# JacksonCampolattaro/spectrogram-rs

Hardware: AMD Instinct MI355X
Metric: STFT frames/sec (4096-pt, hop 256) (higher is better)
Workload: dtype f32

## Files before the change

### bindings/rust/sgx_sys.rs

```rust
use std::os::raw::{c_char, c_int, c_void};

#[repr(C)]
pub struct SgxConfig {
    pub struct_size: u32,
    pub sample_rate: f32, pub period: f32, pub stride: f32,
    pub window_samples: u32, pub hop_samples: u32, pub channels: u32, pub rows: u32,
    pub f_min: f64, pub f_max: f64,
    pub min_db: f32, pub max_db: f32,
    pub interp: u32, pub lut_index_mode: u32,
    pub device: i32, pub flags: u32,
}
#[repr(C)] pub struct SgxCtx { _private: [u8; 0] }
#[repr(C)] pub struct SgxFbank { _private: [u8; 0] }

extern "C" {
    pub fn sgx_config_init(cfg: *mut SgxConfig) -> c_int;
    pub fn sgx_create(cfg: *const SgxConfig, out: *mut *mut SgxCtx) -> c_int;
    pub fn sgx_destroy(ctx: *mut SgxCtx);
    pub fn sgx_last_error(ctx: *const SgxCtx) -> *const c_char;
    pub fn sgx_num_frames(ctx: *const SgxCtx, n_samples: usize) -> usize;
    pub fn sgx_process_one(ctx: *mut SgxCtx, h_lr: *const f32, n_avail: usize, h_out: *mut f32) -> c_int;
    pub fn sgx_stft_batch(ctx: *mut SgxCtx, d_pcm: *const f32, n_samples: usize, first_frame: usize,
                          max_frames: usize, d_mags: *mut f32, n_out: *mut usize) -> c_int;
    pub fn sgx_stft_batch_f16(ctx: *mut SgxCtx, d_pcm: *const f32, n_samples: usize, first_frame: usize,
// ... 28 lines not shown
                            power: u32, out_fbank: *mut *mut SgxFbank) -> c_int;
    pub fn sgx_fbank_destroy(fbank: *mut SgxFbank);
    pub fn sgx_fbank_filters(fbank: *const SgxFbank) -> u32;
    pub fn sgx_fbank_batch(fbank: *mut SgxFbank, d_pcm: *const f32, n_samples: usize, first_frame: usize, max_frames: usize,
                           d_out: *mut f32, n_out: *mut usize) -> c_int;
    pub fn sgx_fbank_mags(fbank: *mut SgxFbank, d_mags: *const f32, n_columns: usize, d_out: *mut f32) -> c_int;
    pub fn sgx_fbank_fused(fbank: *const SgxFbank) -> c_int;
    pub fn sgx_fbank_cross_batch(fbank: *mut SgxFbank, d_pcm: *const f32, n_samples: usize, first_frame: usize, max_frames: usize,
                                 d_out: *mut f32, n_out: *mut usize) -> c_int;
    pub fn sgx_fbank_cross_spec(fbank: *mut SgxFbank, d_spec: *const f32, n_columns: usize, d_out: *mut f32) -> c_int;
    pub fn sgx_fbank_cross_fused(fbank: *const SgxFbank) -> c_int;
    pub fn sgx_mel_weights(sample_rate: f64, window_samples: u32, n_mels: u32, f_min: f64, f_max: f64, scale: u32, norm: u32,
                           h_first: *mut u32, h_count: *mut u32, h_weights: *mut f32, n_weights: *mut usize) -> c_int;
    pub fn sgx_set_gradient(ctx: *mut SgxCtx, h_rgb: *const u8, n: u32, stereo: c_int) -> c_int;
    pub fn sgx_set_gradient_fn(ctx: *mut SgxCtx, eval: extern "C" fn(f64, *mut u8, *mut c_void), user: *mut c_void,
                               stereo: c_int) -> c_int;
    pub fn sgx_set_builtin_scheme(ctx: *mut SgxCtx, name: *const c_char, stereo: c_int) -> c_int;
    pub fn sgx_lookup_table(ctx: *mut SgxCtx, resolution: u32, h_out: *mut f32) -> c_int;
    pub fn sgx_sync(ctx: *mut SgxCtx) -> c_int;
    pub fn sgx_set_cu_limit(ctx: *mut SgxCtx, n: u32) -> c_int;
    pub fn sgx_cu_limit(ctx: *const SgxCtx) -> u32;
    pub fn sgx_set_run_claim(ctx: *mut SgxCtx, static_sixteenths: u32, chunk_jobs: u32) -> c_int;
    pub fn sgx_run_claim(ctx: *const SgxCtx, n_frames: usize, static_sixteenths: *mut u32, chunk_jobs: *mut u32) -> c_int;
}
extern "C" {
    pub fn hipMalloc(p: *mut *mut c_void, bytes: usize) -> c_int;
    pub fn hipFree(p: *mut c_void) -> c_int;
    pub fn hipMemcpy(dst: *mut c_void, src: *const c_void, bytes: usize, kind: c_int) -> c_int;
}
pub const HIP_MEMCPY_HOST_TO_DEVICE: c_int = 1;
pub const HIP_MEMCPY_DEVICE_TO_HOST: c_int = 2;
pub const SGX_FLAG_PAIRED_FRAMES: u32 = 1024;
pub const SGX_FLAG_COMPLEX_MONO: u32 = 512;
pub const SGX_FLAG_LARGE_TRANSFORM: u32 = 4096;
pub const SGX_MEL_HTK: u32 = 0;
pub const SGX_MEL_SLANEY: u32 = 1;
pub const SGX_MEL_NORM_NONE: u32 = 0;
pub const SGX_MEL_NORM_SLANEY: u32 = 1;
pub const SGX_LIVE_BANDS: c_int = 3;
```

### include/sgx.h

```cpp
#ifndef SGX_H
#define SGX_H

#include <stddef.h>
#include <stdint.h>

#ifdef __cplusplus
extern "C" {
#endif

#if defined(__GNUC__)
#define SGX_API __attribute__((visibility("default")))
#else
#define SGX_API
#endif

typedef enum sgx_status {
    SGX_OK = 0,
    SGX_ERR_INVALID_ARG = -1,
    SGX_ERR_UNSUPPORTED = -2,
    SGX_ERR_HIP = -3,
    SGX_ERR_NOMEM = -4,
    SGX_ERR_NO_DEVICE = -5
} sgx_status;

// ... 49 lines not shown


SGX_API const char *sgx_version(void);

SGX_API int sgx_config_init(sgx_config *cfg);

SGX_API int sgx_create(const sgx_config *cfg, sgx_ctx **out_ctx);
SGX_API void sgx_destroy(sgx_ctx *ctx);

SGX_API const char *sgx_last_error(const sgx_ctx *ctx);

SGX_API int sgx_query(const sgx_ctx *ctx, sgx_info *out);

SGX_API size_t sgx_num_frames(const sgx_ctx *ctx, size_t n_samples);

SGX_API int sgx_set_stream(sgx_ctx *ctx, void *stream);
SGX_API int sgx_sync(sgx_ctx *ctx);

SGX_API int sgx_set_cu_limit(sgx_ctx *ctx, uint32_t n);
SGX_API uint32_t sgx_cu_limit(const sgx_ctx *ctx);

SGX_API int sgx_set_run_claim(sgx_ctx *ctx, uint32_t static_sixteenths, uint32_t chunk_jobs);
SGX_API int sgx_run_claim(const sgx_ctx *ctx, size_t n_frames, uint32_t *static_sixteenths, uint32_t *chunk_jobs);


SGX_API int sgx_stft_batch(sgx_ctx *ctx, const float *d_pcm, size_t n_samples, size_t first_frame,
                           size_t max_frames, float *d_mags, size_t *n_out);

SGX_API int sgx_stft_batch_complex(sgx_ctx *ctx, const float *d_pcm, size_t n_samples, size_t first_frame,
                                   size_t max_frames, float *d_spec, size_t *n_out);

SGX_API int sgx_istft_batch(sgx_ctx *ctx, const float *d_spec, size_t n_frames, size_t first_sample,
                            size_t max_samples, float *d_pcm, size_t *n_out);
SGX_API int sgx_istft_supported(const sgx_ctx *ctx);

SGX_API int sgx_stft_batch_f16(sgx_ctx *ctx, const float *d_pcm, size_t n_samples, size_t first_frame,
                               size_t max_frames, void *d_mags_f16, size_t *n_out);

SGX_API int sgx_process_one(sgx_ctx *ctx, const float *h_lr, size_t n_avail, float *h_out);


SGX_API int sgx_render_batch(sgx_ctx *ctx, const float *d_pcm, size_t n_samples, size_t first_frame,
                             size_t max_frames, uint8_t *d_rgba, size_t *n_out);

SGX_API int sgx_render_mags(sgx_ctx *ctx, const float *d_mags, size_t n_columns, uint8_t *d_rgba);

// ... 108 lines not shown
```

### spectrogram_rs_amd/_lib.py

```python
from __future__ import annotations

import ctypes as C
import os

_HERE = os.path.dirname(os.path.abspath(__file__))
LIB_PATH = os.environ.get("SGX_LIB", os.path.join(_HERE, "libsgx.so"))

SGX_OK = 0
SGX_ERR_INVALID_ARG = -1
SGX_ERR_UNSUPPORTED = -2
SGX_ERR_HIP = -3
SGX_ERR_NOMEM = -4
SGX_ERR_NO_DEVICE = -5

INTERP_CUBIC, INTERP_COSINE = 0, 1
LUT_FLOOR_N, LUT_ROUND_NM1 = 0, 1
FLAG_FORCE_GENERIC = 1
FLAG_NO_FUSED_RENDER = 4
FLAG_LUT_WALK = 64
FLAG_MIXED_GENERIC = 256
FLAG_COMPLEX_MONO = 512
FLAG_PAIRED_FRAMES = 1024
FLAG_LARGE_TRANSFORM = 4096
LIVE_MAGS, LIVE_MAGS_F16, LIVE_RGBA, LIVE_BANDS = 0, 1, 2, 3
# ... 44 lines not shown
        ("stft_kernel", C.c_uint32),
        ("render_path", C.c_uint32),
        ("mags_bytes_per_frame", C.c_uint64),
        ("rgba_bytes_per_frame", C.c_uint64),
    ]


_vp, _sz = C.c_void_p, C.c_size_t
_ctx = C.c_void_p
SIGNATURES = [
    ("sgx_version", C.c_char_p, []),
    ("sgx_config_init", C.c_int, [C.POINTER(sgx_config)]),
    ("sgx_create", C.c_int, [C.POINTER(sgx_config), C.POINTER(_ctx)]),
    ("sgx_destroy", None, [_ctx]),
    ("sgx_last_error", C.c_char_p, [_ctx]),
    ("sgx_query", C.c_int, [_ctx, C.POINTER(sgx_info)]),
    ("sgx_num_frames", _sz, [_ctx, _sz]),
    ("sgx_set_stream", C.c_int, [_ctx, _vp]),
    ("sgx_sync", C.c_int, [_ctx]),
    ("sgx_set_cu_limit", C.c_int, [_ctx, C.c_uint32]),
    ("sgx_cu_limit", C.c_uint32, [_ctx]),
    ("sgx_set_run_claim", C.c_int, [_ctx, C.c_uint32, C.c_uint32]),
    ("sgx_run_claim", C.c_int, [_ctx, _sz, C.POINTER(C.c_uint32), C.POINTER(C.c_uint32)]),
    ("sgx_stft_batch", C.c_int, [_ctx, _vp, _sz, _sz, _sz, _vp, C.POINTER(_sz)]),
    ("sgx_stft_batch_f16", C.c_int, [_ctx, _vp, _sz, _sz, _sz, _vp, C.POINTER(_sz)]),
    ("sgx_stft_batch_complex", C.c_int, [_ctx, _vp, _sz, _sz, _sz, _vp, C.POINTER(_sz)]),
    ("sgx_istft_batch", C.c_int, [_ctx, _vp, _sz, _sz, _sz, _vp, C.POINTER(_sz)]),
    ("sgx_istft_supported", C.c_int, [_ctx]),
    ("sgx_process_one", C.c_int, [_ctx, _vp, _sz, _vp]),
    ("sgx_render_batch", C.c_int, [_ctx, _vp, _sz, _sz, _sz, _vp, C.POINTER(_sz)]),
    ("sgx_render_mags", C.c_int, [_ctx, _vp, _sz, _vp]),
    ("sgx_magnitude_in", C.c_int, [_ctx, _vp, _sz, _vp, C.c_uint32, _vp]),
    ("sgx_bands_batch", C.c_int, [_ctx, _vp, _sz, _sz, _sz, _vp, C.POINTER(_sz)]),
    ("sgx_bands_fused", C.c_int, [_ctx]),
    ("sgx_bands_peak_batch", C.c_int, [_ctx, _vp, _sz, _sz, _sz, _sz, _vp, C.POINTER(_sz)]),
    ("sgx_bands_peak_fused", C.c_int, [_ctx]),
    ("sgx_psd_batch", C.c_int, [_ctx, _vp, _sz, _sz, _sz, _sz, _vp, C.POINTER(_sz)]),
    ("sgx_csd_batch", C.c_int, [_ctx, _vp, _sz, _sz, _sz, _sz, _vp, C.POINTER(_sz)]),
    ("sgx_psd_mags", C.c_int, [_ctx, _vp, _sz, _sz, _vp, C.POINTER(_sz)]),
    ("sgx_csd_spec", C.c_int, [_ctx, _vp, _sz, _sz, _vp, C.POINTER(_sz)]),
    ("sgx_psd_fused", C.c_int, [_ctx]),
    ("sgx_csd_fused", C.c_int, [_ctx]),
    ("sgx_render_bands", C.c_int, [_ctx, _vp, _sz, _vp]),
    ("sgx_fbank_create", C.c_int, [_ctx, C.c_uint32, _vp, _vp, _vp, C.c_uint32, C.POINTER(_vp)]),
    ("sgx_fbank_destroy", None, [_vp]),
    ("sgx_fbank_filters", C.c_uint32, [_vp]),
# ... 69 lines not shown
```

### spectrogram_rs_amd/csrc/run_claim.hpp

```cpp
#pragma once

namespace sgx {

struct RunClaim {
    unsigned long long per;
    unsigned long long pool_begin;
    unsigned long long n_chunks;
    unsigned long long chunk;
};
struct JobRun { unsigned long long begin, end; };

inline RunClaim run_claim(unsigned long long n_jobs, unsigned long long blocks, unsigned static_sixteenths, unsigned long long chunk_jobs)
{
    RunClaim r;
    r.per = (n_jobs / 16 * static_sixteenths + n_jobs % 16 * static_sixteenths / 16) / blocks;
    r.pool_begin = blocks * r.per;
    r.chunk = chunk_jobs < 1 ? 1 : chunk_jobs;
    r.n_chunks = (n_jobs - r.pool_begin + r.chunk - 1) / r.chunk;
    return r;
}
inline JobRun static_run(const RunClaim &r, unsigned long long block) { return {block * r.per, (block + 1) * r.per}; }
inline JobRun claimed_run(const RunClaim &r, unsigned long long n_jobs, unsigned long long i)
{
    if (i >= r.n_chunks) return {n_jobs, n_jobs};
    const unsigned long long b = r.pool_begin + i * r.chunk, left = n_jobs - b;
    return {b, b + (left < r.chunk ? left : r.chunk)};
}

constexpr unsigned kClaimAutoSixteenths = 12, kClaimAutoChunk = 8;
constexpr unsigned long long kClaimMinStatic = 64;
inline bool run_claim_engages(unsigned long long n_jobs, unsigned long long blocks)
{
    return run_claim(n_jobs, blocks, kClaimAutoSixteenths, kClaimAutoChunk).per >= kClaimMinStatic;
}
inline bool run_claim_valid(unsigned static_sixteenths, unsigned chunk_jobs)
{
    if (chunk_jobs == 0) return static_sixteenths == 0 || static_sixteenths == 16;
    return static_sixteenths <= 16 && chunk_jobs <= (1u << 20);
}

}
```

### spectrogram_rs_amd/csrc/sgx_internal.hpp

```cpp
#pragma once

#include <hip/hip_runtime.h>

#include <cstdint>
#include <array>
#include <memory>
#include <string>
#include <vector>

#include "../../include/sgx.h"
#include "device_buffer.hpp"
#include "unit_root.hpp"

namespace sgx {

#ifdef __HIPCC__
typedef float sgx_f2v __attribute__((ext_vector_type(2)));
__device__ __forceinline__ float2 cubic_pair(float2 y0, float2 y1, float2 y2, float2 y3, float mu, float mu2, float mu3)
{
    const sgx_f2v Y0 = {y0.x, y0.y}, Y1 = {y1.x, y1.y}, Y2 = {y2.x, y2.y}, Y3 = {y3.x, y3.y};
    const sgx_f2v a0 = ((Y3 - Y2) - Y0) + Y1;
    const sgx_f2v a1 = (Y0 - Y1) - a0;
    const sgx_f2v a2 = Y2 - Y0;
    const sgx_f2v r = ((a0 * mu3) + (a1 * mu2)) + ((a2 * mu) + Y1);
// ... 107 lines not shown
    sgx::TablesPtr<sgx::blu::BluTables> blu;
    sgx::TablesPtr<sgx::mix::MixTables> mix;
    sgx::TablesPtr<sgx::w48::W48Tables> w4800;
    sgx::TablesPtr<sgx::wgr::RealTables> real;
    sgx::TablesPtr<sgx::mix::ChirpTables> chz;
    sgx::TablesPtr<sgx::w16k::TablesW> w16k;
    sgx::TablesPtr<sgx::large::LargeTables> large;
    sgx::TablesPtr<sgx::istft::ITables> istft;

    sgx::DeviceBuffer<float> d_ws_mags;
    sgx::DeviceBuffer<float> d_one_in, d_one_out;
    sgx::DeviceBuffer<unsigned long long> d_cksum;
    std::vector<float> bands_key;
    sgx::DeviceBuffer<sgx::RowEntry> d_band_rows;
    sgx::DeviceBuffer<sgx::SampleEntry> d_band_samples;
    sgx::DeviceBuffer<float> d_levels;
    sgx::DeviceBuffer<double> d_psd_carry;

    unsigned long long palette_gen = 0;

    int n_cu = 256;
    int n_cu_device = 256;
    uint32_t claim_sixteenths = 0, claim_chunk = 0;
    size_t lds_optin = 64 * 1024;
    mutable std::vector<std::pair<std::array<size_t, 3>, int>> occupancy_cache;
    std::vector<struct sgx_view *> views;
    std::vector<struct sgx_image *> images;
    std::vector<struct sgx_fbank *> fbanks;

    std::string err;

    ~sgx_ctx();
};

namespace sgx {

enum class Out { kMags, kMagsF16, kComplex, kRgba, kBands, kPeak, kFbank, kFbankCross, kPsd, kCsd };
struct StftCall {
    const float *pcm;
    uint32_t channels, pairs;
    size_t first, n, total;
    void *out;
    Out kind;
    size_t peak_group;
    const struct sgx_fbank *bank = nullptr;
};
// ... 88 lines not shown
```

### spectrogram_rs_amd/csrc/stft4096_real.hip

```cpp
#include <cmath>
#include <type_traits>

#include "run_claim.hpp"
#include "stft4096_wg.hpp"

namespace sgx {

namespace wgr {

using wg::kBufComplex;
using wg::kLdsBytes;
using wg::kLdsBytesRender;
using wg::kM;
using wg::kS1;
using wg::kS2;
using wg::kW;
using wg::lds_barrier;
using wg::lds_read_alone;
using wg::lds_cfloat2;
using wg::lds_ptr;
using wg::pcm_rsrc;
using wg::u32x2;
using wg::u32x4;

// ... 117 lines not shown
        win[2 * a] = p.window[2 * t_p1 + 512 * a] * (1.0f / 2048.0f);
        win[2 * a + 1] = p.window[2 * t_p1 + 512 * a + 1] * (1.0f / 2048.0f);
    }
    float2 tw1[8];
#pragma unroll
    for (int q = 1; q < 8; ++q) tw1[q] = p.tw1[q * 256 + t_p1];
    const int F = tid >> 7, u = tid & 127;
    float2 twu[8];
#pragma unroll
    for (int q = 0; q < 8; ++q) twu[q] = p.twu[q * 128 + u];
    const int g2 = tid >> 4, t0_2 = tid & 15;
    const int cbase2 = (g2 >> 3) * 128 + (g2 & 7);
    __syncthreads();

#ifdef SGX_VARIANT_SKIP_LAST_JOB
    constexpr bool CLAIM = false;
#else
    constexpr bool CLAIM = !FUSED;
#endif
    const bool claiming = CLAIM && p.claim_counter != nullptr;
    unsigned long long *claim_word = reinterpret_cast<unsigned long long *>(tw2 + 256);
    unsigned long long job_begin = (unsigned long long)blockIdx.x * p.jobs_per_block;
    unsigned long long job_end = job_begin + p.jobs_per_block;
    if (job_end > p.n_jobs) job_end = p.n_jobs;
#ifdef SGX_VARIANT_SKIP_LAST_JOB
    if (job_end > job_begin + 1) --job_end;
#endif
    if (job_begin >= job_end && !claiming) return;

    auto samples_from = [&](unsigned long long first) {
        const unsigned long long left = first < p.stream_samples ? (p.stream_samples - first) * 4 : 0;
        const unsigned long long addr = (unsigned long long)(p.pcm + (first < p.stream_samples ? first : 0));
        const uint32_t lo = __builtin_amdgcn_readfirstlane((uint32_t)addr), hi = __builtin_amdgcn_readfirstlane((uint32_t)(addr >> 32));
        const int records = __builtin_amdgcn_readfirstlane((int)(left < 0x7fffffffull ? left : 0x7fffffffull));
        return __builtin_amdgcn_make_buffer_rsrc(reinterpret_cast<void *>(((unsigned long long)hi << 32) | lo), 0, records, 0x00020000);
    };
    auto columns_from = [&](unsigned long long col0) { return samples_from(2 * col0); };
    auto column = [&](__amdgpu_buffer_rsrc_t r, int byte_offset) {
        const u32x2 v = __builtin_amdgcn_raw_buffer_load_b64(r, t_p1 * 8, byte_offset, 0);
        return make_float2(__uint_as_float(v.x), __uint_as_float(v.y));
    };
    float2 R[8];
    float2 L;
    auto load_pair = [&](unsigned long long fa_) {
        const __amdgpu_buffer_rsrc_t r0 = samples_from(fa_ * p.H), r1 = samples_from((fa_ + 1) * p.H);
#pragma unroll
// ... 339 lines not shown
    for (int q = 0; q < 8; ++q)
        for (int tt = 0; tt < 256; ++tt) tw1[q * 256 + tt] = unit_root2((unsigned long long)tt * q, 2048);
    for (int q = 0; q < 16; ++q)
        for (int t0 = 0; t0 < 16; ++t0) tw2[q * 16 + t0] = unit_root2((unsigned long long)t0 * q, 256);
    for (int q3 = 0; q3 < 8; ++q3)
        for (int uu = 0; uu < 128; ++uu) twu[q3 * 128 + uu] = unit_root2((unsigned long long)(uu + 128 * q3), 4096);
    twu[0] = unit_root2(1024, 4096);
    hipError_t e = t->d_tw1.upload(tw1);
    if (e == hipSuccess) e = t->d_tw2.upload(tw2);
    if (e == hipSuccess) e = t->d_twu.upload(twu);
    if (e == hipSuccess) e = t->d_claim.alloc(1);
    if (e == hipSuccess) c->real = std::move(t);
    return e;
}

bool real4096_serves(const sgx_ctx *c, const float *d_pcm, uint32_t channels)
{
    (void)d_pcm;
    return channels == 1 && c->real && c->W == (uint32_t)wgr::kW;
}

namespace wg {

struct RowsClaim { uint32_t sixteenths, chunk; };
static RowsClaim rows_claim(const sgx_ctx *c, Out kind, unsigned long long n_jobs, unsigned long long blocks)
{
    const bool rows = kind == Out::kMags || kind == Out::kMagsF16 || kind == Out::kComplex;
#ifdef SGX_VARIANT_SKIP_LAST_JOB
    const bool compiled = false;
#else
    const bool compiled = true;
#endif
    if (!rows || !compiled || n_jobs == 0 || (c->claim_sixteenths == 16u && c->claim_chunk == 0u)) return {16u, 0u};
    if (c->claim_chunk != 0u) return {c->claim_sixteenths, c->claim_chunk};
    if (kind == Out::kComplex) return {16u, 0u};
    return run_claim_engages(n_jobs, blocks) ? RowsClaim{kClaimAutoSixteenths, kClaimAutoChunk} : RowsClaim{16u, 0u};
}

hipError_t launch_real4096(const sgx_ctx *c, Params p, Out kind)
{
    using namespace wgr;
    if (p.n_frames == 0) return hipSuccess;
    const RealTables *t = c->real.get();
    const bool hold_peak = kind == Out::kPeak;
    p.tw1 = t->d_tw1.get();
    p.tw2 = t->d_tw2.get();
    p.twu = t->d_twu.get();
    p.stream_samples = p.total_frames ? (p.total_frames - 1) * (unsigned long long)c->H + (unsigned long long)kW : 0;
    p.n_jobs = (p.n_frames + 1) / 2;
    RunSplit runs = run_split(c, p.n_jobs, 4);
    if (hold_peak) {
        runs = runs_of(p.n_jobs, peak_align_run(runs.per, 2, p.peak_group));
        p.peak_run = 2 * runs.per;
    }
    p.jobs_per_block = runs.per;
    const RowsClaim rc = rows_claim(c, kind, p.n_jobs, runs.blocks);
    if (rc.sixteenths != 16u || rc.chunk != 0u) {
        const RunClaim split = run_claim(p.n_jobs, runs.blocks, rc.sixteenths, rc.chunk);
        const hipError_t e = hipMemsetAsync(t->d_claim.get(), 0, sizeof(unsigned long long), c->stream);
        if (e != hipSuccess) return e;
        p.jobs_per_block = split.per;
        p.claim_counter = t->d_claim.get();
        p.claim_pool_begin = split.pool_begin;
        p.claim_chunks = split.n_chunks;
        p.claim_chunk = (uint32_t)split.chunk;
    }
    const size_t lds_claim = p.claim_counter ? sizeof(unsigned long long) : 0;
    const dim3 grid((unsigned)runs.blocks), block(256);
    auto launch = [&](auto slide_c) {
        constexpr bool S_ = decltype(slide_c)::value;
        const size_t lds_rows = (S_ ? kLdsBytesR : kLdsBytes) + lds_claim;
        constexpr size_t lds_render = S_ ? kLdsBytesRenderR : kLdsBytesRender;
        if (hold_peak) {
            if (p.interp == SGX_INTERP_COSINE) hipLaunchKernelGGL((stft4096_real_kernel<kPeak, kPixPeakCosine, S_>), grid, block, lds_rows, c->stream, p);
            else hipLaunchKernelGGL((stft4096_real_kernel<kPeak, kPixPeakCubic, S_>), grid, block, lds_rows, c->stream, p);
        } else if (kind == Out::kFbank) {
            hipLaunchKernelGGL((stft4096_real_kernel<kFbank, kPixFbank, S_>), grid, block, lds_rows, c->stream, p);
        } else if (kind == Out::kBands) {
            if (p.interp == SGX_INTERP_COSINE) hipLaunchKernelGGL((stft4096_real_kernel<kBands, kPixBandsCosine, S_>), grid, block, lds_rows, c->stream, p);
            else hipLaunchKernelGGL((stft4096_real_kernel<kBands, kPixBandsCubic, S_>), grid, block, lds_rows, c->stream, p);
        } else if (kind == Out::kRgba) {
            if (!p.seed_pm1) hipLaunchKernelGGL((stft4096_real_kernel<kPixels, kPixGeneric, S_>), grid, block, lds_render, c->stream, p);
            else if (p.interp == SGX_INTERP_COSINE) hipLaunchKernelGGL((stft4096_real_kernel<kPixels, kPixCosine, S_>), grid, block, lds_render, c->stream, p);
            else hipLaunchKernelGGL((stft4096_real_kernel<kPixels, kPixCubic, S_>), grid, block, lds_render, c->stream, p);
// ... 10 lines not shown
    const hipError_t e = hipGetLastError();
    return e == hipSuccess && hold_peak ? launch_peak_combine(c, p, runs.blocks) : e;
}

}

}

int sgx_set_run_claim(sgx_ctx *c, uint32_t static_sixteenths, uint32_t chunk_jobs)
{
    if (!c) return SGX_ERR_INVALID_ARG;
    if (!sgx::run_claim_valid(static_sixteenths, chunk_jobs)) {
        c->err = "sgx_set_run_claim: a share of 0 .. 16 sixteenths with a chunk of 1 .. 2^20 jobs, (16, 0) for the static split or (0, 0) for the automatic rule";
        return SGX_ERR_INVALID_ARG;
    }
    c->claim_sixteenths = static_sixteenths;
    c->claim_chunk = chunk_jobs;
    return SGX_OK;
}

int sgx_run_claim(const sgx_ctx *c, size_t n_frames, uint32_t *static_sixteenths, uint32_t *chunk_jobs)
{
    if (!c || !static_sixteenths || !chunk_jobs) return SGX_ERR_INVALID_ARG;
    sgx::wg::RowsClaim rc{16u, 0u};
    if (sgx::real4096_serves(c, nullptr, c->C) && !(c->cfg.flags & (SGX_FLAG_PAIRED_FRAMES | SGX_FLAG_COMPLEX_MONO))) {
        const unsigned long long n_jobs = ((unsigned long long)n_frames + 1) / 2;
        rc = sgx::wg::rows_claim(c, sgx::Out::kMags, n_jobs, sgx::run_split(c, n_jobs, 4).blocks);
    }
    *static_sixteenths = rc.sixteenths;
    *chunk_jobs = rc.chunk;
    return SGX_OK;
}
```

### spectrogram_rs_amd/csrc/stft4096_wg.hip

```cpp
#include <cmath>
#include <type_traits>

#include "stft4096_wg.hpp"

namespace sgx {

namespace wg {

typedef float f2v __attribute__((ext_vector_type(2)));
__device__ __forceinline__ float cl_fma(float a, float c, float u) { return fmaf(a, c, u); }
__device__ __forceinline__ f2v cl_fma(f2v a, float c, f2v u) { return __builtin_elementwise_fma(a, f2v{c, c}, u); }

#include "fft_codelets.inc"

__device__ __forceinline__ float2 cmulf(float2 a, float2 b)
{
    return make_float2(fmaf(a.x, b.x, -(a.y * b.y)), fmaf(a.x, b.y, a.y * b.x));
}

constexpr int kPrioA = 1, kPrioB = 2;
#if SGX_STAMPS
__device__ unsigned long long g_phase_cycles[20];
#endif

__device__ __forceinline__ void addtid_rows(float2 a, float2 b, uint32_t m0_wave, int q)
{
    asm volatile("s_mov_b32 m0, %4\n\t"
                 "s_nop 0\n\t"
                 "ds_write_addtid_b32 %0 offset:%5\n\t"
                 "ds_write_addtid_b32 %1 offset:%6\n\t"
                 "ds_write_addtid_b32 %2 offset:%7\n\t"
                 "ds_write_addtid_b32 %3 offset:%8"
                 :
                 : "v"(a.x), "v"(a.y), "v"(b.x), "v"(b.y), "s"(m0_wave), "i"(1088 * q), "i"(1088 * q + 17408), "i"(1088 * (q + 1)), "i"(1088 * (q + 1) + 17408)
                 : "memory");
}
__device__ __forceinline__ void read_planes(const float4 *rd4, float (&xr)[16], float (&xi)[16])
{
#pragma unroll
    for (int c = 0; c < 4; ++c) {
        const float4 r = rd4[c], i = rd4[c + 1088];
        xr[4 * c] = r.x; xr[4 * c + 1] = r.y; xr[4 * c + 2] = r.z; xr[4 * c + 3] = r.w;
        xi[4 * c] = i.x; xi[4 * c + 1] = i.y; xi[4 * c + 2] = i.z; xi[4 * c + 3] = i.w;
    }
}
// ... 2 lines not shown
__global__ void __launch_bounds__(256, 4) stft4096_wg_kernel(Params p)
{
    constexpr bool C64 = PIX == kPixRowsC64;
    constexpr bool RENDER = PIX != kPixNone && PIX != kPixRowsF16 && !C64;
    constexpr bool BANDS = pix_bands(PIX);
    constexpr bool F16 = PIX == kPixRowsF16;
    constexpr bool FBANK = PIX == kPixFbank;
    static_assert(!(FBANK && MONO), "paired mono frames take the workspace route of sgx_fbank_batch");
    constexpr bool CROSS = PIX == kPixFbankCross;
    static_assert(!CROSS || (!MONO && C2), "the cross sums need a pair: (l, r) streams and pair planes only");
    extern __shared__ __attribute__((aligned(16))) unsigned char smem_raw[];
    float2 *buf = reinterpret_cast<float2 *>(smem_raw);
    float2 *tw2 = buf + kBufComplex;

    uint2 *pal = reinterpret_cast<uint2 *>(tw2 + 256);

    const int tid = threadIdx.x;
    constexpr bool kSlide2 = !MONO && C2 && PAIRING == kPairAdjacentRow;
    constexpr bool TR = kSlide2;
    const int t_p1 = TR ? (tid >> 4) + 16 * (tid & 15) : tid;
    float *plane = reinterpret_cast<float *>(smem_raw);
    const uint32_t m0_wave = __builtin_amdgcn_readfirstlane((uint32_t)(tid >> 6) * 272u);
    const float4 *rd4 = reinterpret_cast<const float4 *>(plane + 272 * (tid >> 4) + 68 * ((tid & 15) >> 2) + 16 * (tid & 3));
    tw2[tid] = p.tw2[tid];
    uint32_t row_words[4] = {0u, 0u, 0u, 0u};
    if (RENDER && !FBANK && !CROSS) {
        if (!BANDS) pal[tid] = make_uint2(__float_as_uint(tid < 255 ? p.lut_thr[tid] : __builtin_nanf("")), *reinterpret_cast<const uint32_t *>(&p.lut_rgba[tid]));
#pragma unroll
        for (int i = 0; i < 4; ++i)
            if ((uint32_t)tid + 256u * i < p.R) row_words[i] = p.rows[tid + 256 * i];
    }

    const float inv_w = 1.0f / (float)kW;
    static_assert((kW & (kW - 1)) == 0, "the scale must be a power of two to move it");
    float win[8];
#pragma unroll
    for (int a = 0; a < 8; ++a) win[a] = p.window[t_p1 + 256 * a] * inv_w;
    float2 tw1[16];
#pragma unroll
    for (int q = 1; q < 16; ++q) tw1[q] = p.tw1[q * 256 + t_p1];

    const int q1_2 = tid >> 4, t0_2 = tid & 15;
    __syncthreads();

    const unsigned long long job_begin = (unsigned long long)blockIdx.x * p.jobs_per_block;
    unsigned long long job_end = job_begin + p.jobs_per_block;
// ... 337 lines not shown
                float2 *dst_b = bands + ((size_t)f1 * p.pairs + p.pair) * (size_t)p.R;
                __builtin_amdgcn_s_setprio(3);
                row_pass_bands<MONO>(p, row_words, vbuf, dst_a, dst_b, have_first, have_second, tid);
            } else {
                lds_barrier();
                uchar4 *rgba = reinterpret_cast<uchar4 *>(p.rgba);
                uchar4 *dst_a = rgba + ((size_t)(have_first ? f0 : 0) * p.pairs + p.pair) * (size_t)p.R;
                uchar4 *dst_b = rgba + ((size_t)f1 * p.pairs + p.pair) * (size_t)p.R;
                __builtin_amdgcn_s_setprio(3);
                row_pass<MONO, PIX>(p, row_words, vbuf, dst_a, dst_b, have_first, have_second, pal, tid);
            }
            }
        }
        SGX_STAMP(13)
        if (!RENDER && !(MONO && PAIRING == kPairAdjacentRow && kSlideWindow)) next_samples_are_here();
        if (kSlide2) {
#pragma unroll
            for (int a = 0; a < 7; ++a) { sa[a] = sa[a + 1]; sb[a] = sb[a + 1]; }
            sa[7] = ld0;
            sb[7] = ld1;
        }
    }
#if SGX_STAMPS
    if ((tid & 63) == 0) {
#pragma unroll
        for (int i = 0; i < 16; ++i) atomicAdd(&g_phase_cycles[i], st_acc[i]);
        atomicAdd(&g_phase_cycles[16], (unsigned long long)(job_end > job_begin ? job_end - job_begin : 0));
    }
#endif
}

__global__ void __launch_bounds__(256) peak_combine_kernel(const float2 *partial, float2 *out, unsigned long long n_frames, unsigned long long group,
                                                           unsigned long long run, uint32_t R, uint32_t pairs, uint32_t pair)
{
    const unsigned long long b = (unsigned long long)blockIdx.x + 1, fb = b * run;
    const unsigned long long j = fb / group, c0 = j * group;
    if (c0 == fb) return;
    const unsigned long long b_lo = c0 / run;
    if (b_lo + 1 != b) return;
    unsigned long long c1 = c0 + group;
    if (c1 > n_frames) c1 = n_frames;
    const unsigned long long b_hi = (c1 - 1) / run;
    const uint32_t py = blockIdx.y * 256 + threadIdx.x;
    if (py >= R) return;
    float2 m = partial[(b_lo * 2 + 1) * R + py];
    for (unsigned long long bb = b; bb <= b_hi; ++bb) {
// ... 19 lines not shown
    size_t zeros = 0;
    for (size_t e = 0; e < lut_thr.size(); ++e) {
        const float t = lut_thr[e];
        if (!(t == t) || t < 0.0f || !std::isfinite(t)) return false;
        if (e > 0 && t < lut_thr[e - 1]) return false;
        if (t == 0.0f) { zeros = e + 1; continue; }
        const double ue = u((double)t);
        if (!(ue > (double)e + 0.51 && ue < (double)e + 1.49)) return false;
    }
    return u(0.0) > (double)zeros - 0.49;
}

}

#if SGX_STAMPS
extern "C" __attribute__((visibility("default"))) int sgx_debug_phase_cycles(unsigned long long *h_out, int reset)
{
    hipError_t e = hipMemcpyFromSymbol(h_out, HIP_SYMBOL(wg::g_phase_cycles), sizeof(unsigned long long) * 20);
    if (e == hipSuccess && reset) {
        unsigned long long zero[20] = {0};
        e = hipMemcpyToSymbol(HIP_SYMBOL(wg::g_phase_cycles), zero, sizeof(zero));
    }
    return e == hipSuccess ? 0 : -1;
}
#endif

void TablesDelete::operator()(wg::WgTables *t) const { delete t; }

hipError_t wg4096_init(sgx_ctx *c)
{
    using namespace wg;
    TablesPtr<WgTables> t(new WgTables());
    std::vector<float2> tw1(16 * 256), tw2(256);
    for (int q = 0; q < 16; ++q)
        for (int tt = 0; tt < 256; ++tt) tw1[q * 256 + tt] = unit_root2(tt * q, kP);
    for (int q = 0; q < 16; ++q)
        for (int t0 = 0; t0 < 16; ++t0) tw2[q * 16 + t0] = unit_root2(t0 * q, 256);

    std::vector<uint32_t> rows(c->tab.rows.size());
    std::vector<PackedSample> samples;
    bool fusable = c->tab.rows.size() <= 1024;
    auto packed = [&](const SampleEntry &se) {
        PackedSample ps;
        ps.i0 = se.i0;
        ps.w = c->cfg.interp == SGX_INTERP_COSINE ? se.w2 : se.w0;
        if (se.i0 < 0 || se.i0 > (int32_t)c->M - 1) fusable = false;
// ... 213 lines not shown
```

### spectrogram_rs_amd/csrc/stft4096_wg.hpp

```cpp
#pragma once
#include <hip/hip_fp16.h>

#include "sgx_fbank.hpp"
#include "sgx_internal.hpp"

namespace sgx {
namespace wg {

constexpr int kW = 2048, kP = 4096, kM = 2047;
constexpr bool kSlideWindow = true;
constexpr int kS1 = 272;
constexpr int kS2 = 257;
constexpr int kBufComplex = 16 * kS1;
constexpr size_t kLdsBytes = (size_t)(kBufComplex + 256) * sizeof(float2);
constexpr size_t kLdsBytesRender = kLdsBytes + 256 * sizeof(uint2);

struct PackedSample {
    int32_t i0;
    float w;
};

struct Params {
    const float *pcm;
    const float2 *tw1;
// ... 3 lines not shown
        float *mags;
        float2 *peak_partial;
    };
    unsigned long long first_frame, n_frames, n_jobs, jobs_per_block;
    unsigned long long pair_base;
    unsigned long long total_frames;
    uint32_t H, C, pair_l, pair_r, pairs, pair;
    uint32_t out_f16;
    union {
        const uint32_t *rows;
        unsigned long long *claim_counter;
    };
    union {
        const PackedSample *samples;
        unsigned long long claim_pool_begin;
    };
    union {
        uint32_t n_samples;
        uint32_t claim_chunk;
    };
    union {
        const float *lut_thr;
        unsigned long long peak_group;
    };
    union {
        const uchar4 *lut_rgba;
        unsigned long long peak_run;
    };
    union {
        uint8_t *rgba;
        unsigned long long claim_chunks;
    };
    uint32_t R, interp;
    float guess_a, guess_b;
    uint32_t seed_pm1;
    uint32_t single_rows;
    uint32_t block_max_cnt;
    const float2 *twu;
    unsigned long long stream_samples;
};
static_assert(sizeof(Params) == 216, "the kernel argument of every instantiation: its size is part of their code objects");

inline unsigned long long peak_align_run(unsigned long long per, unsigned fpj, unsigned long long group)
{
    const unsigned long long unit = group % fpj == 0 ? group : group * fpj, run = per * fpj;
    if (unit > run / 32) return per;
    return (run + unit - 1) / unit * unit / fpj;
}
hipError_t launch_peak_combine(const sgx_ctx *c, const Params &p, unsigned long long blocks);

hipError_t launch_real4096(const sgx_ctx *c, Params p, Out kind);

constexpr int kPairAdjacentRow = 0, kPairAdjacent = 1;

struct WgTables {
    DeviceBuffer<float2> d_tw1, d_tw2;
    DeviceBuffer<uint32_t> d_rows;
    DeviceBuffer<PackedSample> d_samples;
    uint32_t n_samples = 0;
// ... 400 lines not shown
```

### spectrogram_rs_amd/engine.py

```python
from __future__ import annotations

import ctypes as C
from typing import Optional

import numpy as np

from . import _lib
from ._lib import SgxError, sgx_config, sgx_info


class SpectrogramEngine:
    def __init__(self, sample_rate: float = 48000.0, *, period: float = 0.0, stride: float = 0.0,
                 window_samples: int = 0, hop_samples: int = 0, channels: int = 1, rows: int = 1024,
                 f_min: float = 32.0, f_max: float = 22030.0, min_db: float = -70.0, max_db: float = -10.0,
                 interp: int = _lib.INTERP_CUBIC, lut_index_mode: int = _lib.LUT_FLOOR_N,
                 device: Optional[int] = None, force_generic: bool = False, gradient: Optional[str] = None,
                 fused_render: bool = True, lut_walk: bool = False,
                 mixed_generic: bool = False, complex_mono: bool = False, paired_frames: bool = False,
                 large_transforms: bool = False):
        import torch

        self._lib = _lib.load()
        self._ctx = C.c_void_p()
        cfg = sgx_config()
# ... 65 lines not shown
        self._check(self._lib.sgx_set_stream(self._ctx, C.c_void_p(s.cuda_stream)))

    def set_stream(self, cuda_stream: int):
        self._check(self._lib.sgx_set_stream(self._ctx, C.c_void_p(cuda_stream)))

    def sync(self):
        self._check(self._lib.sgx_sync(self._ctx))

    def set_cu_limit(self, n: int):
        self._check(self._lib.sgx_set_cu_limit(self._ctx, C.c_uint32(n)))

    @property
    def cu_limit(self) -> int:
        return int(self._lib.sgx_cu_limit(self._ctx))

    def set_run_claim(self, static_sixteenths: int, chunk_jobs: int):
        self._check(self._lib.sgx_set_run_claim(self._ctx, C.c_uint32(static_sixteenths), C.c_uint32(chunk_jobs)))

    def run_claim(self, n_frames: int):
        s, k = C.c_uint32(), C.c_uint32()
        self._check(self._lib.sgx_run_claim(self._ctx, C.c_size_t(n_frames), C.byref(s), C.byref(k)))
        return int(s.value), int(k.value)

    def _dev_f32(self, t):
        import torch

        assert isinstance(t, torch.Tensor) and t.is_cuda and t.dtype == torch.float32 and t.is_contiguous(), \
            "expected a contiguous float32 CUDA tensor"
        assert t.device == self.device, f"tensor on {t.device}, engine on {self.device}"
        return C.c_void_p(t.data_ptr())

    def _out(self, out, shape, dtype):
        import torch

        self.use_current_stream()
        if out is None:
            return torch.empty(shape, dtype=dtype, device=self.device)
        need = 1
        for d in shape:
            need *= int(d)
        assert isinstance(out, torch.Tensor) and out.is_cuda and out.device == self.device, \
            f"out must be a CUDA tensor on {self.device}"
        assert out.dtype == dtype, f"out must be {dtype}, got {out.dtype}"
        assert out.is_contiguous(), "out must be contiguous"
        assert out.numel() >= need, f"out holds {out.numel()} elements, the call writes {need}"
        return out
# ... 625 lines not shown
```

Measured before the change: 304.5 million.

## Weight static job runs by dispatch slot so later block waves get fewer jobs

Adds a slot-weighted static job split for the 4096-point real STFT kernel. Blocks are grouped into four slots by dispatch order (multiples of the CU count), and each slot gets a different per-block job count from built-in weights, with earlier slots getting more. The remaining jobs go to the atomic claim pool. The aim is to reduce tail imbalance, where later-launched blocks finish last, and the auto weights are hardcoded for hop 256 with no CU limit. It reuses Params union fields for the slot data and adds debug finish-time stamps plus an API to set or query the weights.

```diff
diff --git a/bindings/rust/sgx_sys.rs b/bindings/rust/sgx_sys.rs
--- a/bindings/rust/sgx_sys.rs
+++ b/bindings/rust/sgx_sys.rs
@@ -74,6 +74,8 @@
     pub fn sgx_cu_limit(ctx: *const SgxCtx) -> u32;
     pub fn sgx_set_run_claim(ctx: *mut SgxCtx, static_sixteenths: u32, chunk_jobs: u32) -> c_int;
     pub fn sgx_run_claim(ctx: *const SgxCtx, n_frames: usize, static_sixteenths: *mut u32, chunk_jobs: *mut u32) -> c_int;
+    pub fn sgx_set_run_weights(ctx: *mut SgxCtx, w: *const u32) -> c_int;
+    pub fn sgx_run_weights(ctx: *const SgxCtx, n_frames: usize, w: *mut u32) -> c_int;
 }
 extern "C" {
     pub fn hipMalloc(p: *mut *mut c_void, bytes: usize) -> c_int;
diff --git a/include/sgx.h b/include/sgx.h
--- a/include/sgx.h
+++ b/include/sgx.h
@@ -95,6 +95,8 @@
 
 SGX_API int sgx_set_run_claim(sgx_ctx *ctx, uint32_t static_sixteenths, uint32_t chunk_jobs);
 SGX_API int sgx_run_claim(const sgx_ctx *ctx, size_t n_frames, uint32_t *static_sixteenths, uint32_t *chunk_jobs);
+SGX_API int sgx_set_run_weights(sgx_ctx *ctx, const uint32_t w[4]);
+SGX_API int sgx_run_weights(const sgx_ctx *ctx, size_t n_frames, uint32_t w[4]);
 
 
 SGX_API int sgx_stft_batch(sgx_ctx *ctx, const float *d_pcm, size_t n_samples, size_t first_frame,
diff --git a/spectrogram_rs_amd/_lib.py b/spectrogram_rs_amd/_lib.py
--- a/spectrogram_rs_amd/_lib.py
+++ b/spectrogram_rs_amd/_lib.py
@@ -90,6 +90,8 @@
     ("sgx_cu_limit", C.c_uint32, [_ctx]),
     ("sgx_set_run_claim", C.c_int, [_ctx, C.c_uint32, C.c_uint32]),
     ("sgx_run_claim", C.c_int, [_ctx, _sz, C.POINTER(C.c_uint32), C.POINTER(C.c_uint32)]),
+    ("sgx_set_run_weights", C.c_int, [_ctx, C.POINTER(C.c_uint32)]),
+    ("sgx_run_weights", C.c_int, [_ctx, _sz, C.POINTER(C.c_uint32)]),
     ("sgx_stft_batch", C.c_int, [_ctx, _vp, _sz, _sz, _sz, _vp, C.POINTER(_sz)]),
     ("sgx_stft_batch_f16", C.c_int, [_ctx, _vp, _sz, _sz, _sz, _vp, C.POINTER(_sz)]),
     ("sgx_stft_batch_complex", C.c_int, [_ctx, _vp, _sz, _sz, _sz, _vp, C.POINTER(_sz)]),
diff --git a/spectrogram_rs_amd/csrc/run_claim.hpp b/spectrogram_rs_amd/csrc/run_claim.hpp
--- a/spectrogram_rs_amd/csrc/run_claim.hpp
+++ b/spectrogram_rs_amd/csrc/run_claim.hpp
@@ -39,4 +39,58 @@
     return static_sixteenths <= 16 && chunk_jobs <= (1u << 20);
 }
 
+struct SlotDeal {
+    unsigned long long per[4];
+    unsigned long long n_cu;
+    unsigned long long leftover;
+    RunClaim claim;
+};
+constexpr unsigned long long slot_of(unsigned long long block, unsigned long long n_cu) { return block / n_cu < 3 ? block / n_cu : 3; }
+constexpr unsigned long long slot_blocks(unsigned long long blocks, unsigned long long n_cu, unsigned s)
+{
+    const unsigned long long lo = s * n_cu;
+    return blocks <= lo ? 0 : (s == 3 || blocks - lo < n_cu ? blocks - lo : n_cu);
 }
+constexpr bool run_weights_valid(const unsigned w[4]) { return w[0] >= 1 && w[1] >= 1 && w[2] >= 1 && w[3] >= 1 && w[0] <= 256 && w[1] <= 256 && w[2] <= 256 && w[3] <= 256 && w[0] + w[1] + w[2] + w[3] == 256; }
+constexpr SlotDeal slot_deal(unsigned long long n_jobs, unsigned long long blocks, unsigned long long n_cu, unsigned static_sixteenths, unsigned long long chunk_jobs,
+                             const unsigned w[4])
+{
+    SlotDeal d{};
+    const unsigned long long T = static_sixteenths >= 16 ? n_jobs : n_jobs / 16 * static_sixteenths + n_jobs % 16 * static_sixteenths / 16;
+    unsigned long long den = 0, dealt = 0;
+    for (unsigned s = 0; s < 4; ++s) den += slot_blocks(blocks, n_cu, s) * w[s];
+    for (unsigned s = 0; s < 4; ++s) {
+        d.per[s] = T * w[s] / den;
+        dealt += slot_blocks(blocks, n_cu, s) * d.per[s];
+    }
+    d.n_cu = n_cu;
+    d.leftover = static_sixteenths >= 16 ? n_jobs - dealt : 0;
+    d.claim.per = T / blocks;
+    d.claim.chunk = chunk_jobs < 1 ? 1 : chunk_jobs;
+    d.claim.pool_begin = static_sixteenths >= 16 ? n_jobs : dealt;
+    d.claim.n_chunks = (n_jobs - d.claim.pool_begin + d.claim.chunk - 1) / d.claim.chunk;
+    return d;
+}
+constexpr JobRun slot_run(const SlotDeal &d, unsigned long long block)
+{
+    const unsigned s = (block >= d.n_cu ? 1u : 0u) + (block >= 2 * d.n_cu ? 1u : 0u) + (block >= 3 * d.n_cu ? 1u : 0u);
+    const unsigned long long before = (s > 0 ? d.per[0] : 0) + (s > 1 ? d.per[1] : 0) + (s > 2 ? d.per[2] : 0);
+    const unsigned long long per = s == 0 ? d.per[0] : s == 1 ? d.per[1] : s == 2 ? d.per[2] : d.per[3];
+    const unsigned long long begin = d.n_cu * before + (block - s * d.n_cu) * per + (block < d.leftover ? block : d.leftover);
+    return {begin, begin + per + (block < d.leftover ? 1 : 0)};
+}
+constexpr JobRun weighted_run(unsigned long long n_jobs, unsigned long long blocks, unsigned long long n_cu, unsigned static_sixteenths, unsigned long long chunk_jobs,
+                              const unsigned w[4], unsigned long long block)
+{
+    return slot_run(slot_deal(n_jobs, blocks, n_cu, static_sixteenths, chunk_jobs, w), block);
+}
+
+constexpr unsigned kSlotWeightsEqual[4] = {64, 64, 64, 64};
+constexpr unsigned kSlotWeightsAuto[4] = {80, 73, 56, 47};
+constexpr unsigned kSlotWeightsAutoComplex[4] = {86, 72, 53, 45};
+constexpr const unsigned *slot_weights_auto(bool complex_rows) { return complex_rows ? kSlotWeightsAutoComplex : kSlotWeightsAuto; }
+constexpr unsigned kSlotAutoSixteenths = 15, kSlotAutoChunk = 4;
+constexpr bool slot_weights_measured(unsigned long long blocks, unsigned long long n_cu, bool cu_limited, unsigned hop = 256) { return hop == 256 && !cu_limited && blocks > 3 * n_cu; }
+constexpr bool slot_weights_equal(const unsigned w[4]) { return w[0] == 64 && w[1] == 64 && w[2] == 64 && w[3] == 64; }
+
+}
diff --git a/spectrogram_rs_amd/csrc/sgx_internal.hpp b/spectrogram_rs_amd/csrc/sgx_internal.hpp
--- a/spectrogram_rs_amd/csrc/sgx_internal.hpp
+++ b/spectrogram_rs_amd/csrc/sgx_internal.hpp
@@ -153,6 +153,7 @@
     int n_cu = 256;
     int n_cu_device = 256;
     uint32_t claim_sixteenths = 0, claim_chunk = 0;
+    uint32_t run_weights[4] = {0, 0, 0, 0};
     size_t lds_optin = 64 * 1024;
     mutable std::vector<std::pair<std::array<size_t, 3>, int>> occupancy_cache;
     std::vector<struct sgx_view *> views;
diff --git a/spectrogram_rs_amd/csrc/stft4096_real.hip b/spectrogram_rs_amd/csrc/stft4096_real.hip
--- a/spectrogram_rs_amd/csrc/stft4096_real.hip
+++ b/spectrogram_rs_amd/csrc/stft4096_real.hip
@@ -163,6 +163,19 @@
     unsigned long long *claim_word = reinterpret_cast<unsigned long long *>(tw2 + 256);
     unsigned long long job_begin = (unsigned long long)blockIdx.x * p.jobs_per_block;
     unsigned long long job_end = job_begin + p.jobs_per_block;
+    if (CLAIM && p.slot_n_cu != 0u) {
+        SlotDeal deal{};
+        deal.per[0] = p.slot_per0;
+        deal.per[1] = p.slot_per1;
+        deal.per[2] = ((unsigned long long)p.slot_per2_hi << 32) | p.slot_per2_lo;
+        deal.per[3] = ((unsigned long long)p.slot_per3_hi << 32) | p.slot_per3_lo;
+        deal.n_cu = p.slot_n_cu;
+        deal.leftover = p.slot_leftover;
+        const JobRun run = slot_run(deal, blockIdx.x);
+        auto uniform = [](unsigned long long v) { return ((unsigned long long)__builtin_amdgcn_readfirstlane((uint32_t)(v >> 32)) << 32) | __builtin_amdgcn_readfirstlane((uint32_t)v); };
+        job_begin = uniform(run.begin);
+        job_end = uniform(run.end);
+    }
     if (job_end > p.n_jobs) job_end = p.n_jobs;
 #ifdef SGX_VARIANT_SKIP_LAST_JOB
     if (job_end > job_begin + 1) --job_end;
@@ -548,7 +561,7 @@
 
 namespace wg {
 
-struct RowsClaim { uint32_t sixteenths, chunk; };
+struct RowsClaim { uint32_t sixteenths, chunk; uint32_t w[4]; };
 static RowsClaim rows_claim(const sgx_ctx *c, Out kind, unsigned long long n_jobs, unsigned long long blocks)
 {
     const bool rows = kind == Out::kMags || kind == Out::kMagsF16 || kind == Out::kComplex;
@@ -557,10 +570,22 @@
 #else
     const bool compiled = true;
 #endif
-    if (!rows || !compiled || n_jobs == 0 || (c->claim_sixteenths == 16u && c->claim_chunk == 0u)) return {16u, 0u};
-    if (c->claim_chunk != 0u) return {c->claim_sixteenths, c->claim_chunk};
-    if (kind == Out::kComplex) return {16u, 0u};
-    return run_claim_engages(n_jobs, blocks) ? RowsClaim{kClaimAutoSixteenths, kClaimAutoChunk} : RowsClaim{16u, 0u};
+    RowsClaim rc{16u, 0u, {64u, 64u, 64u, 64u}};
+    if (!rows || !compiled || n_jobs == 0) return rc;
+    const bool forced_w = c->run_weights[0] != 0u;
+    const unsigned *w = forced_w ? c->run_weights : slot_weights_measured(blocks, (unsigned long long)c->n_cu, c->n_cu != c->n_cu_device, c->H) ? slot_weights_auto(kind == Out::kComplex) : kSlotWeightsEqual;
+    for (int s = 0; s < 4; ++s) rc.w[s] = w[s];
+    if (c->claim_sixteenths == 16u && c->claim_chunk == 0u) return rc;
+    if (c->claim_chunk != 0u) {
+        rc.sixteenths = c->claim_sixteenths;
+        rc.chunk = c->claim_chunk;
+        return rc;
+    }
+    if (kind == Out::kComplex || !run_claim_engages(n_jobs, blocks)) return rc;
+    const bool weighted = !slot_weights_equal(rc.w);
+    rc.sixteenths = weighted ? kSlotAutoSixteenths : kClaimAutoSixteenths;
+    rc.chunk = weighted ? kSlotAutoChunk : kClaimAutoChunk;
+    return rc;
 }
 
 hipError_t launch_real4096(const sgx_ctx *c, Params p, Out kind)
@@ -581,11 +606,26 @@
     }
     p.jobs_per_block = runs.per;
     const RowsClaim rc = rows_claim(c, kind, p.n_jobs, runs.blocks);
-    if (rc.sixteenths != 16u || rc.chunk != 0u) {
-        const RunClaim split = run_claim(p.n_jobs, runs.blocks, rc.sixteenths, rc.chunk);
+    const bool pooled = rc.sixteenths != 16u || rc.chunk != 0u;
+    RunClaim split{};
+    if (!slot_weights_equal(rc.w)) {
+        const SlotDeal deal = slot_deal(p.n_jobs, runs.blocks, (unsigned long long)c->n_cu, rc.sixteenths, rc.chunk, rc.w);
+        p.slot_per0 = deal.per[0];
+        p.slot_per1 = deal.per[1];
+        p.slot_per2_lo = (uint32_t)deal.per[2];
+        p.slot_per2_hi = (uint32_t)(deal.per[2] >> 32);
+        p.slot_per3_lo = (uint32_t)deal.per[3];
+        p.slot_per3_hi = (uint32_t)(deal.per[3] >> 32);
+        p.slot_n_cu = (uint32_t)c->n_cu;
+        p.slot_leftover = (uint32_t)deal.leftover;
+        split = deal.claim;
+    } else if (pooled) {
+        split = run_claim(p.n_jobs, runs.blocks, rc.sixteenths, rc.chunk);
+        p.jobs_per_block = split.per;
+    }
+    if (pooled) {
         const hipError_t e = hipMemsetAsync(t->d_claim.get(), 0, sizeof(unsigned long long), c->stream);
         if (e != hipSuccess) return e;
-        p.jobs_per_block = split.per;
         p.claim_counter = t->d_claim.get();
         p.claim_pool_begin = split.pool_begin;
         p.claim_chunks = split.n_chunks;
@@ -642,7 +682,7 @@
 int sgx_run_claim(const sgx_ctx *c, size_t n_frames, uint32_t *static_sixteenths, uint32_t *chunk_jobs)
 {
     if (!c || !static_sixteenths || !chunk_jobs) return SGX_ERR_INVALID_ARG;
-    sgx::wg::RowsClaim rc{16u, 0u};
+    sgx::wg::RowsClaim rc{16u, 0u, {64u, 64u, 64u, 64u}};
     if (sgx::real4096_serves(c, nullptr, c->C) && !(c->cfg.flags & (SGX_FLAG_PAIRED_FRAMES | SGX_FLAG_COMPLEX_MONO))) {
         const unsigned long long n_jobs = ((unsigned long long)n_frames + 1) / 2;
         rc = sgx::wg::rows_claim(c, sgx::Out::kMags, n_jobs, sgx::run_split(c, n_jobs, 4).blocks);
@@ -651,3 +691,27 @@
     *chunk_jobs = rc.chunk;
     return SGX_OK;
 }
+
+int sgx_set_run_weights(sgx_ctx *c, const uint32_t *w)
+{
+    if (!c) return SGX_ERR_INVALID_ARG;
+    const bool automatic = !w || (w[0] == 0u && w[1] == 0u && w[2] == 0u && w[3] == 0u);
+    if (!automatic && !sgx::run_weights_valid(w)) {
+        c->err = "sgx_set_run_weights: four weights of at least 1 each that sum to 256, or all zero (a null pointer) for the automatic ones";
+        return SGX_ERR_INVALID_ARG;
+    }
+    for (int s = 0; s < 4; ++s) c->run_weights[s] = automatic ? 0u : w[s];
+    return SGX_OK;
+}
+
+int sgx_run_weights(const sgx_ctx *c, size_t n_frames, uint32_t *w)
+{
+    if (!c || !w) return SGX_ERR_INVALID_ARG;
+    sgx::wg::RowsClaim rc{16u, 0u, {64u, 64u, 64u, 64u}};
+    if (sgx::real4096_serves(c, nullptr, c->C) && !(c->cfg.flags & (SGX_FLAG_PAIRED_FRAMES | SGX_FLAG_COMPLEX_MONO))) {
+        const unsigned long long n_jobs = ((unsigned long long)n_frames + 1) / 2;
+        rc = sgx::wg::rows_claim(c, sgx::Out::kMags, n_jobs, sgx::run_split(c, n_jobs, 4).blocks);
+    }
+    for (int s = 0; s < 4; ++s) w[s] = rc.w[s];
+    return SGX_OK;
+}
diff --git a/spectrogram_rs_amd/csrc/stft4096_wg.hip b/spectrogram_rs_amd/csrc/stft4096_wg.hip
--- a/spectrogram_rs_amd/csrc/stft4096_wg.hip
+++ b/spectrogram_rs_amd/csrc/stft4096_wg.hip
@@ -21,6 +21,12 @@
 constexpr int kPrioA = 1, kPrioB = 2;
 #if SGX_STAMPS
 __device__ unsigned long long g_phase_cycles[20];
+constexpr int kFinishBlocks = 4096;
+__device__ unsigned long long g_finish[4 * kFinishBlocks];
+#if SGX_STAMPS == 2
+#undef SGX_STAMP
+#define SGX_STAMP(i)
+#endif
 #endif
 
 __device__ __forceinline__ void addtid_rows(float2 a, float2 b, uint32_t m0_wave, int q)
@@ -69,6 +75,9 @@
     float *plane = reinterpret_cast<float *>(smem_raw);
     const uint32_t m0_wave = __builtin_amdgcn_readfirstlane((uint32_t)(tid >> 6) * 272u);
     const float4 *rd4 = reinterpret_cast<const float4 *>(plane + 272 * (tid >> 4) + 68 * ((tid & 15) >> 2) + 16 * (tid & 3));
+#if SGX_STAMPS
+    if (tid == 0 && blockIdx.x < kFinishBlocks) g_finish[4 * blockIdx.x] = wall_clock64();
+#endif
     tw2[tid] = p.tw2[tid];
     uint32_t row_words[4] = {0u, 0u, 0u, 0u};
     if (RENDER && !FBANK && !CROSS) {
@@ -452,6 +461,11 @@
         }
     }
 #if SGX_STAMPS
+    if (tid == 0 && blockIdx.x < kFinishBlocks) {
+        g_finish[4 * blockIdx.x + 1] = wall_clock64();
+        g_finish[4 * blockIdx.x + 2] = blockIdx.x;
+        g_finish[4 * blockIdx.x + 3] = job_end > job_begin ? job_end - job_begin : 0;
+    }
     if ((tid & 63) == 0) {
 #pragma unroll
         for (int i = 0; i < 16; ++i) atomicAdd(&g_phase_cycles[i], st_acc[i]);
@@ -517,6 +531,11 @@
         e = hipMemcpyToSymbol(HIP_SYMBOL(wg::g_phase_cycles), zero, sizeof(zero));
     }
     return e == hipSuccess ? 0 : -1;
+}
+extern "C" __attribute__((visibility("default"))) int sgx_debug_finish(unsigned long long *h_out, int n_blocks)
+{
+    if (n_blocks < 0 || n_blocks > wg::kFinishBlocks) return -1;
+    return hipMemcpyFromSymbol(h_out, HIP_SYMBOL(wg::g_finish), sizeof(unsigned long long) * 4 * (size_t)n_blocks) == hipSuccess ? 0 : -1;
 }
 #endif
 
diff --git a/spectrogram_rs_amd/csrc/stft4096_wg.hpp b/spectrogram_rs_amd/csrc/stft4096_wg.hpp
--- a/spectrogram_rs_amd/csrc/stft4096_wg.hpp
+++ b/spectrogram_rs_amd/csrc/stft4096_wg.hpp
@@ -49,19 +49,23 @@
     union {
         const float *lut_thr;
         unsigned long long peak_group;
+        unsigned long long slot_per0;
     };
     union {
         const uchar4 *lut_rgba;
         unsigned long long peak_run;
+        unsigned long long slot_per1;
     };
     union {
         uint8_t *rgba;
         unsigned long long claim_chunks;
     };
-    uint32_t R, interp;
-    float guess_a, guess_b;
-    uint32_t seed_pm1;
-    uint32_t single_rows;
+    union { uint32_t R; uint32_t slot_per2_lo; };
+    union { uint32_t interp; uint32_t slot_per2_hi; };
+    union { float guess_a; uint32_t slot_per3_lo; };
+    union { float guess_b; uint32_t slot_per3_hi; };
+    union { uint32_t seed_pm1; uint32_t slot_n_cu; };
+    union { uint32_t single_rows; uint32_t slot_leftover; };
     uint32_t block_max_cnt;
     const float2 *twu;
     unsigned long long stream_samples;
diff --git a/spectrogram_rs_amd/engine.py b/spectrogram_rs_amd/engine.py
--- a/spectrogram_rs_amd/engine.py
+++ b/spectrogram_rs_amd/engine.py
@@ -111,6 +111,15 @@
         self._check(self._lib.sgx_run_claim(self._ctx, C.c_size_t(n_frames), C.byref(s), C.byref(k)))
         return int(s.value), int(k.value)
 
+    def set_run_weights(self, w=None):
+        arr = (C.c_uint32 * 4)(*(int(x) for x in w)) if w is not None else None
+        self._check(self._lib.sgx_set_run_weights(self._ctx, arr))
+
+    def run_weights(self, n_frames: int):
+        w = (C.c_uint32 * 4)()
+        self._check(self._lib.sgx_run_weights(self._ctx, C.c_size_t(n_frames), w))
+        return tuple(int(x) for x in w)
+
     def _dev_f32(self, t):
         import torch
 
```

Result: faster. 313.4 million, median of 6 (+2.9%).
